# msg7086/x265-Yuuki-Asuna

Measured on AMD Instinct MI355X. Metric: encoded fps + bit-exact check, 4K preset=slow, 1/2/4/8 MI355X vs host AVX2, higher is better.
Workload: dtype u8; 1 GPU; 3840x2160 8-bit closed-loop frame pipeline (tier T2): lookahead -> exhaustive +-57 ME, 85 PUs/CTU -> subme 3 -> MC + DCT/quant/recon qp 27 -> deblock -> SAO (rdo) -> border -> next reference; parallelism=none (1 GPU), ctus_per_frame=2040

## Files before the change

### include/x265hip.h

```cpp
#ifndef X265HIP_H
#define X265HIP_H

#include <stdint.h>
#include <stddef.h>

#ifdef __cplusplus
extern "C" {
#endif

#define X265HIP_ME_PUS_PER_CTU 85
#define X265HIP_OK            0
#define X265HIP_ENODEV       -1
#define X265HIP_EINVAL       -2
#define X265HIP_EUNSUPPORTED -3
#define X265HIP_EBUSY        -4

const char* x265hip_version(void);
int x265hip_stream_release(void* stream);
const char* x265hip_last_error(void);
int         x265hip_device_count(void);
int         x265hip_init(int device);
#define X265HIP_WAIT_BLOCK 0
#define X265HIP_WAIT_SPIN  1
int         x265hip_set_wait_policy(int policy);
// ... 39 lines not shown
static inline size_t x265hip_surf_ctu_bytes(int surf_format, int range)
{
    const size_t nc = (size_t)(2 * range + 1), recs = nc * ((nc + 3) >> 2);
    if (surf_format == X265HIP_SURF_I32) return recs * X265HIP_SURF_GROUP_BYTES_I32;
    if (surf_format == X265HIP_SURF_PACKED_B) return ((recs + 63) >> 6) * X265HIP_SURF_BLOCK_BYTES_PACKED;
    return recs * X265HIP_SURF_GROUP_BYTES_PACKED;
}
int x265hip_me_fullsearch(const x265hip_me_params* p, void* stream);
int x265hip_me_best_reset(uint64_t* best, size_t count, void* stream);
const char* x265hip_me_minima_kernel_name(int depth, int range);
void x265hip_me_env_refresh(void);

typedef struct x265hip_subpel_params
{
    int depth;
    int width, height;
    int range;
    int subme;
    const void* fenc;  intptr_t fenc_stride;
    const void* fref;  intptr_t fref_stride;
    const uint64_t* best_in;
    const uint16_t* cost_q;  int qoff;
    void* out;
    const void* phase_planes;  intptr_t phase_plane_samples;
} x265hip_subpel_params;
int x265hip_subpel_refine(const x265hip_subpel_params* p, void* stream);

typedef struct x265hip_subpel_chroma
{
    const void* fenc_cb; const void* fenc_cr; intptr_t fenc_stride_c;
    const void* fref_cb; const void* fref_cr; intptr_t fref_stride_c;
} x265hip_subpel_chroma;
int x265hip_subpel_refine_chroma(const x265hip_subpel_params* p, const x265hip_subpel_chroma* c, void* stream);

#define X265HIP_TU_INTRA_SLICE 1
#define X265HIP_TU_SIGN_HIDE   2
typedef struct x265hip_tu_tables
{
    const int32_t* quant_coeff;
    const int32_t* dequant_coeff;
    const uint16_t* nr_offset;
    uint32_t* nr_residual_sum;
    int16_t* dct_coeff_out;
    int32_t* delta_u_out;
    int64_t* rdoq_cost_uncoded;
    int64_t* rdoq_cg_cost;
    int16_t* rdoq_levels;
    uint32_t* rdoq_num_sig;
    int16_t* fenc_dct_out;
    int64_t psy_scale;
} x265hip_tu_tables;
typedef struct x265hip_recon_params
{
    int depth;
    int width, height;
    int level;
    int qp, intra_slice;
    const void* fenc;  intptr_t fenc_stride;
    const void* fref;  intptr_t fref_stride;
    void* recon;       intptr_t recon_stride;
    const void* mv;
    int16_t* levels; uint32_t* num_sig; uint64_t* dist;
    const x265hip_tu_tables* tables;
    const int8_t* qp_map;
} x265hip_recon_params;
int x265hip_inter_recon(const x265hip_recon_params* p, void* stream);
// ... 787 lines not shown
```

### x265-yuuki-asuna_amd/csrc/subpel_kernels.hip

```cpp
#include "common.h"
#include "tile_interp.h"

namespace x265hip {

struct SubpelArgs
{
    const uint8_t* fenc; long fencStrideB;
    const uint8_t* fref; long frefStrideB;
    int ctusW, range, depth;
    const unsigned long long* bestIn;
    const uint16_t* costQ; int qoff;
    int hpelIters, hpelDirs, qpelIters, qpelDirs, hpelSatd;
    int2* out;
    const uint8_t* planes; long planeBytes;
};

struct SubpelChromaArgs
{
    const uint8_t* fencC[2]; long fencStrideCB;
    const uint8_t* frefC[2]; long frefStrideCB;
};

__constant__ int16_t kSpLumaTaps[4][8] = {
    { 0, 0, 0, 64, 0, 0, 0, 0 }, { -1, 4, -10, 58, 17, -5, 1, 0 },
    { -1, 4, -11, 40, 40, -11, 4, -1 }, { 0, 1, -5, 17, 58, -10, 4, -1 } };
__constant__ int kSpSquare1[9][2] = { { 0, 0 }, { 0, -1 }, { 0, 1 }, { -1, 0 }, { 1, 0 }, { -1, -1 }, { -1, 1 }, { 1, -1 }, { 1, 1 } };

constexpr int SP_MARGIN = 7;

__device__ __forceinline__ int sp_clip16(int v, int maxVal)
{
    const int16_t s = (int16_t)v;
    return s < 0 ? 0 : (s > maxVal ? maxVal : s);
}

struct SpShared
{
    int cost[64][9];
    int best[64], qx[64], qy[64], ix[64], iy[64], state[64];
};

template <typename Px, int LEVEL> struct SpGeom
{
    static constexpr int BPP = sizeof(Px);
    static constexpr int N = 8 << LEVEL, NPU = 64 >> (2 * LEVEL);
    static constexpr int TSHIFT = 2 * LEVEL + 2, NTILES = 1 << TSHIFT, TPR = N >> 2;
    static constexpr int PW = N + 2 * SP_MARGIN + 1;
// ... 318 lines not shown
        {
            const int qx0 = sh.qx[tid], qy0 = sh.qy[tid];
            if (isRem)
                sh.best[tid] = sh.cost[tid][0] + mvcost(qx0, qy0);
            else
            {
                int bcost = sh.best[tid], bdir = 0;
                for (int i = 1; i <= last; i++)
                {
                    const int c = sh.cost[tid][i] + mvcost(qx0 + kSpSquare1[i][0] * step, qy0 + kSpSquare1[i][1] * step);
                    if (c < bcost) { bcost = c; bdir = i; }
                }
                sh.best[tid] = bcost;
                if (bdir) { sh.qx[tid] = qx0 + kSpSquare1[bdir][0] * step; sh.qy[tid] = qy0 + kSpSquare1[bdir][1] * step; }
                else sh.state[tid] = 2;
            }
        }
        if (G::NTILES == 256) { __syncthreads(); if (tid < 9) sh.cost[0][tid] = 0; }
        __syncthreads();
    }
    if (tid < NPU)
    {
        int bcost = sh.best[tid];
        if (sh.state[tid] == 0) bcost = mvcost(sh.qx[tid], sh.qy[tid]);
        a.out[(size_t)ctu * 85 + G::LBASE + tid] = make_int2(bcost, (sh.qx[tid] & 0xffff) | (sh.qy[tid] << 16));
    }
}

template <typename Px, bool PL = false>
__global__ void __launch_bounds__(256) subpel_refine_kernel(SubpelArgs a)
{
    extern __shared__ __attribute__((aligned(16))) uint8_t smemRaw[];
    __shared__ SpShared sh;
    switch (blockIdx.y)
    {
    case 0: subpel_level<Px, 0, PL>(a, smemRaw, sh); break;
    case 1: subpel_level<Px, 1, PL>(a, smemRaw, sh); break;
    case 2: subpel_level<Px, 2, PL>(a, smemRaw, sh); break;
    default: subpel_level<Px, 3, PL>(a, smemRaw, sh); break;
    }
}

template <typename Px, bool PL>
__global__ void __launch_bounds__(256) subpel_refine_chroma_kernel(SubpelArgs a, SubpelChromaArgs ca)
{
    extern __shared__ __attribute__((aligned(16))) uint8_t smemRaw[];
    __shared__ SpShared sh;
    switch (blockIdx.y)
    {
    case 0: subpel_level<Px, 0, PL, true>(a, smemRaw, sh, ca); break;
    case 1: subpel_level<Px, 1, PL, true>(a, smemRaw, sh, ca); break;
    case 2: subpel_level<Px, 2, PL, true>(a, smemRaw, sh, ca); break;
    default: subpel_level<Px, 3, PL, true>(a, smemRaw, sh, ca); break;
    }
}

}

using namespace x265hip;

extern "C" int x265hip_subpel_refine(const x265hip_subpel_params* p, void* stream)
{
    return x265hip_subpel_refine_chroma(p, nullptr, stream);
}

extern "C" int x265hip_subpel_refine_chroma(const x265hip_subpel_params* p, const x265hip_subpel_chroma* c, void* stream)
{
    if (!p || !p->fenc || !p->fref || !p->best_in || !p->cost_q || !p->out) { set_error("subpel_refine: NULL operand"); return X265HIP_EINVAL; }
    if ((p->width & 63) || (p->height & 63) || p->width <= 0 || p->height <= 0) { set_error("subpel_refine: width/height must be multiples of 64"); return X265HIP_EINVAL; }
    if (p->depth != 8 && p->depth != 10 && p->depth != 12) { set_error("subpel_refine: depth %d", p->depth); return X265HIP_EINVAL; }
    if (p->subme < 0 || p->subme > 7) { set_error("subpel_refine: subme %d out of [0,7]", p->subme); return X265HIP_EINVAL; }
    if (p->phase_planes && p->phase_plane_samples <= 0) { set_error("subpel_refine: phase_plane_samples"); return X265HIP_EINVAL; }
    if (c)
    {
        if (!c->fenc_cb || !c->fenc_cr || !c->fref_cb || !c->fref_cr) { set_error("subpel_refine_chroma: NULL chroma plane"); return X265HIP_EINVAL; }
        if (c->fenc_stride_c <= 0 || c->fref_stride_c <= 0) { set_error("subpel_refine_chroma: chroma strides must be positive"); return X265HIP_EINVAL; }
    }
    int rc = ensure_device();
    if (rc) return rc;
    static const int wl[8][5] = { { 1, 4, 0, 4, 0 }, { 1, 4, 1, 4, 0 }, { 1, 4, 1, 4, 1 }, { 2, 4, 1, 4, 1 },
                                  { 2, 4, 2, 4, 1 }, { 1, 8, 1, 8, 1 }, { 2, 8, 1, 8, 1 }, { 2, 8, 2, 8, 1 } };
    const int bpp = p->depth == 8 ? 1 : 2;
    SubpelArgs a;
    a.fenc = (const uint8_t*)p->fenc; a.fencStrideB = (long)p->fenc_stride * bpp;
    a.fref = (const uint8_t*)p->fref; a.frefStrideB = (long)p->fref_stride * bpp;
    a.ctusW = p->width / 64; a.range = p->range; a.depth = p->depth;
    a.bestIn = (const unsigned long long*)p->best_in; a.costQ = p->cost_q; a.qoff = p->qoff;
    a.hpelIters = wl[p->subme][0]; a.hpelDirs = wl[p->subme][1]; a.qpelIters = wl[p->subme][2]; a.qpelDirs = wl[p->subme][3]; a.hpelSatd = wl[p->subme][4];
    a.out = (int2*)p->out;
    a.planes = (const uint8_t*)p->phase_planes; a.planeBytes = (long)p->phase_plane_samples * bpp;
    const int nctu = a.ctusW * (p->height / 64);
    hipStream_t s = (hipStream_t)stream;
    const size_t lds = (size_t)(bpp == 1 ? SpGeom<uint8_t, 0>::PSZ : SpGeom<uint16_t, 0>::PSZ) * 64 * bpp;
    static_assert(SpGeom<uint8_t, 0>::PSZ * 64 >= SpGeom<uint8_t, 1>::PSZ * 16 && SpGeom<uint8_t, 0>::PSZ * 64 >= SpGeom<uint8_t, 2>::PSZ * 4
                  && SpGeom<uint8_t, 0>::PSZ * 64 >= SpGeom<uint8_t, 3>::PSZ, "level 0 is the largest");
    static_assert(SpGeom<uint16_t, 0>::PSZ * 64 >= SpGeom<uint16_t, 1>::PSZ * 16 && SpGeom<uint16_t, 0>::PSZ * 64 >= SpGeom<uint16_t, 2>::PSZ * 4
                  && SpGeom<uint16_t, 0>::PSZ * 64 >= SpGeom<uint16_t, 3>::PSZ, "level 0 is the largest");
    if (c && p->subme >= 3)
    {
        SubpelChromaArgs ca;
        ca.fencC[0] = (const uint8_t*)c->fenc_cb; ca.fencC[1] = (const uint8_t*)c->fenc_cr; ca.fencStrideCB = (long)c->fenc_stride_c * bpp;
        ca.frefC[0] = (const uint8_t*)c->fref_cb; ca.frefC[1] = (const uint8_t*)c->fref_cr; ca.frefStrideCB = (long)c->fref_stride_c * bpp;
        if (a.planes)
        {
            if (p->depth == 8) hipLaunchKernelGGL((subpel_refine_chroma_kernel<uint8_t, true>), dim3(nctu, 4), dim3(256), 0, s, a, ca);
            else hipLaunchKernelGGL((subpel_refine_chroma_kernel<uint16_t, true>), dim3(nctu, 4), dim3(256), 0, s, a, ca);
        }
        else if (p->depth == 8)
            hipLaunchKernelGGL((subpel_refine_chroma_kernel<uint8_t, false>), dim3(nctu, 4), dim3(256), lds, s, a, ca);
        else
        {
            static bool attrC = false;
            if (!attrC) { X265HIP_TRY(hipFuncSetAttribute((const void*)subpel_refine_chroma_kernel<uint16_t, false>, hipFuncAttributeMaxDynamicSharedMemorySize, (int)lds)); attrC = true; }
            hipLaunchKernelGGL((subpel_refine_chroma_kernel<uint16_t, false>), dim3(nctu, 4), dim3(256), lds, s, a, ca);
        }
    }
    else if (a.planes)
    {
        if (p->depth == 8) hipLaunchKernelGGL((subpel_refine_kernel<uint8_t, true>), dim3(nctu, 4), dim3(256), 0, s, a);
        else hipLaunchKernelGGL((subpel_refine_kernel<uint16_t, true>), dim3(nctu, 4), dim3(256), 0, s, a);
    }
    else if (p->depth == 8)
        hipLaunchKernelGGL(subpel_refine_kernel<uint8_t>, dim3(nctu, 4), dim3(256), lds, s, a);
    else
    {
        static bool attr = false;
        if (!attr) { X265HIP_TRY(hipFuncSetAttribute((const void*)subpel_refine_kernel<uint16_t>, hipFuncAttributeMaxDynamicSharedMemorySize, (int)lds)); attr = true; }
        hipLaunchKernelGGL(subpel_refine_kernel<uint16_t>, dim3(nctu, 4), dim3(256), lds, s, a);
    }
    X265HIP_TRY(hipGetLastError());
    return 0;
}
```

### x265-yuuki-asuna_amd/hipabi.py

```python
from __future__ import annotations

import ctypes
import os

_HERE = os.path.dirname(os.path.abspath(__file__))
LIB_PATH = os.path.join(_HERE, "libx265hip.so")

CMP_SAD, CMP_SATD, CMP_SA8D, CMP_SSE_PP, CMP_PSY_COST = range(5)

_lib = None


class X265HipError(RuntimeError):
    pass


class MEParams(ctypes.Structure):
    _fields_ = [
        ("depth", ctypes.c_int), ("width", ctypes.c_int), ("height", ctypes.c_int), ("range", ctypes.c_int),
        ("fenc", ctypes.c_void_p), ("fenc_stride", ctypes.c_ssize_t),
        ("fref", ctypes.c_void_p), ("fref_stride", ctypes.c_ssize_t),
        ("surf", ctypes.c_void_p), ("best", ctypes.c_void_p),
        ("cost_x", ctypes.c_void_p), ("cost_y", ctypes.c_void_p),
        ("surf_format", ctypes.c_int),
# ... 208 lines not shown
def exported_symbols():
    import re
    hdr = os.path.join(os.path.dirname(_HERE), "include", "x265hip.h")
    text = open(hdr).read()
    inline = set(re.findall(r"static inline [^\n(]*\b(x265hip_[a-z0-9_]+)\s*\(", text))
    return sorted(set(re.findall(r"\b(x265hip_[a-z0-9_]+)\s*\(", text)) - inline)


def current_stream() -> int:
    import torch
    return torch.cuda.current_stream().cuda_stream


def _p(t):
    return None if t is None else t.data_ptr()


def me_fullsearch(depth, width, height, rng, fenc, fenc_stride, fref, fref_stride,
                  surf=None, best=None, cost_x=None, cost_y=None,
                  fenc_off=0, fref_off=0, stream=None, surf_format=SURF_I32, centres=None):
    es = 1 if depth == 8 else 2
    p = MEParams()
    p.surf_format = surf_format
    p.depth, p.width, p.height, p.range = depth, width, height, rng
    p.fenc, p.fenc_stride = fenc.data_ptr() + fenc_off * es, fenc_stride
    p.fref, p.fref_stride = fref.data_ptr() + fref_off * es, fref_stride
    p.surf, p.best = _p(surf), _p(best)
    p.cost_x, p.cost_y = _p(cost_x), _p(cost_y)
    p.centres = _p(centres)
    s = current_stream() if stream is None else stream
    check(lib().x265hip_me_fullsearch(ctypes.byref(p), s), "x265hip_me_fullsearch")


def subpel_refine(depth, width, height, rng, subme, fenc, fenc_stride, fref, fref_stride, best_in, cost_q, qoff, out,
                  fenc_off=0, fref_off=0, stream=None, phase_planes=None, chroma=None):
    es = 1 if depth == 8 else 2
    p = SubpelParams()
    p.depth, p.width, p.height, p.range, p.subme = depth, width, height, rng, subme
    p.fenc, p.fenc_stride = fenc.data_ptr() + fenc_off * es, fenc_stride
    p.fref, p.fref_stride = fref.data_ptr() + fref_off * es, fref_stride
    p.best_in, p.cost_q, p.qoff, p.out = best_in.data_ptr(), cost_q.data_ptr(), qoff, out.data_ptr()
    if phase_planes is not None:
        p.phase_planes, p.phase_plane_samples = phase_planes.data_ptr() + fref_off * es, fref.numel() * fref.element_size() // es
    s = current_stream() if stream is None else stream
    if chroma is not None:
        c = SubpelChroma()
        c.fenc_cb, c.fenc_cr = (t.data_ptr() + chroma["fenc_org"] * es for t in chroma["fenc"])
        c.fref_cb, c.fref_cr = (t.data_ptr() + chroma["fref_org"] * es for t in chroma["fref"])
        c.fenc_stride_c, c.fref_stride_c = chroma["fenc_stride"], chroma["fref_stride"]
        f = lib().x265hip_subpel_refine_chroma
        f.argtypes = [ctypes.POINTER(SubpelParams), ctypes.POINTER(SubpelChroma), ctypes.c_void_p]
        check(f(ctypes.byref(p), ctypes.byref(c), s), "x265hip_subpel_refine_chroma")
        return
    f = lib().x265hip_subpel_refine
    f.argtypes = [ctypes.POINTER(SubpelParams), ctypes.c_void_p]
    check(f(ctypes.byref(p), s), "x265hip_subpel_refine")


def bidir_decide(depth, width, height, level, fenc, fenc_stride, fref0, fref1, fref_stride, mv0, mv1, cost_q, qoff, dir_cost, dir_out, mv0_out, mv1_out,
                 ref0=None, ref1=None, cost_out=None, ref_ids=(0, 1), fenc_off=0, fref_off=0, phase_planes=None, stream=None, chroma=None):
    es = 1 if depth == 8 else 2
    p = BidirParams()
    p.depth, p.width, p.height, p.level = depth, width, height, level
    p.fenc, p.fenc_stride = fenc.data_ptr() + fenc_off * es, fenc_stride
    p.fref0, p.fref1, p.fref_stride = fref0.data_ptr() + fref_off * es, fref1.data_ptr() + fref_off * es, fref_stride
    p.mv0, p.mv1, p.cost_q, p.qoff = mv0.data_ptr(), mv1.data_ptr(), cost_q.data_ptr(), qoff
    p.dir_cost[0], p.dir_cost[1], p.dir_cost[2] = (int(c) for c in dir_cost)
    p.ref_id0, p.ref_id1 = ref_ids
    if phase_planes is not None:
        p.phase_planes0, p.phase_planes1 = (t.data_ptr() + fref_off * es for t in phase_planes)
        p.phase_plane_samples = fref0.numel() * fref0.element_size() // es
    p.dir, p.ref0, p.ref1 = dir_out.data_ptr(), _p(ref0), _p(ref1)
    p.mv0_out, p.mv1_out, p.cost_out = mv0_out.data_ptr(), mv1_out.data_ptr(), _p(cost_out)
    s = current_stream() if stream is None else stream
    if chroma is not None:
        c = BidirChroma()
        c.fenc_cb, c.fenc_cr = (t.data_ptr() + chroma["fenc_org"] * es for t in chroma["fenc"])
        c.fref0_cb, c.fref0_cr = (t.data_ptr() + chroma["fref_org"] * es for t in chroma["fref0"])
        c.fref1_cb, c.fref1_cr = (t.data_ptr() + chroma["fref_org"] * es for t in chroma["fref1"])
        c.fenc_stride_c, c.fref_stride_c = chroma["fenc_stride"], chroma["fref_stride"]
        f = lib().x265hip_bidir_decide_chroma
        f.argtypes = [ctypes.POINTER(BidirParams), ctypes.POINTER(BidirChroma), ctypes.c_void_p]
# ... 994 lines not shown
```

### x265-yuuki-asuna_amd/pipeline.py

```python
from __future__ import annotations

import numpy as np

from . import frames as F
from . import hipabi

LEVEL_SIZES = (8, 16, 32, 64)
LEVEL_PUS = (64, 16, 4, 1)
LEVEL_BASE = (0, 64, 80, 84)
PUS_PER_CTU = 85


class DevicePicture:

    def __init__(self, img: np.ndarray, device, cb: np.ndarray = None, cr: np.ndarray = None):
        import torch
        buf, self.stride, self.org, self.w64, self.h64 = F.pad_plane(img)
        self.depth = 8 if img.dtype == np.uint8 else 10

        def up(b):
            return torch.from_numpy(b if b.dtype == np.uint8 else b.view(np.int16)).to(device)
        self.t = up(buf)
        self.host = buf
        self.c, self.c_host, self.stride_c, self.org_c = None, None, 0, 0
# ... 134 lines not shown
            out["surf"] = int(sum(self.level_view(l)[0].sum(dtype=torch.int64).item() for l in range(4)))
        return out


class SubpelRefine:

    def __init__(self, ms: MotionSearch, subme: int, device, lam=4.0, phase_planes=False, chroma_satd=False):
        import torch
        self.ms, self.subme = ms, subme
        self.chroma_satd = bool(chroma_satd)
        self.use_planes, self.planes = bool(phase_planes), None
        cq, self.qoff = F.qpel_cost_table(ms.range, lam)
        self.cost_q_host = cq
        self.cost_q = torch.from_numpy(cq.view(np.int16)).to(device)
        self.out = torch.zeros(ms.nctu * PUS_PER_CTU * 2, dtype=torch.int32, device=device)

    def part(self, ms_part, ctu_row0):
        import copy
        o = copy.copy(self)
        o.ms, o.parent = ms_part, self
        c0 = (ms_part.w64 // 64) * ctu_row0
        o.out = self.out[c0 * PUS_PER_CTU * 2:(c0 + ms_part.nctu) * PUS_PER_CTU * 2]
        return o

    def prepare(self, ref: DevicePicture):
        import torch
        if not self.use_planes:
            return
        nb = ref.t.numel() * ref.t.element_size()
        if self.planes is None or self.planes.numel() != 15 * nb:
            self.planes = torch.empty(15 * nb, dtype=torch.uint8, device=ref.t.device)
        hipabi.phase_planes(self.ms.depth, ref.t, 0, self.planes, ref.stride, nb // (ref.stride * (1 if self.ms.depth == 8 else 2)))

    def run(self, cur: DevicePicture, ref: DevicePicture, prepared=False):
        ms = self.ms
        if not prepared:
            self.prepare(ref)
        planes = getattr(self, "parent", self).planes if self.use_planes else None
        chroma = None
        if self.chroma_satd:
            if cur.c is None or ref.c is None:
                raise ValueError("SubpelRefine(chroma_satd=True) needs pictures with chroma planes")
            if (4 * ms.range + 6 + 7) // 8 + 6 > min(F.CHROMA_MARGIN_X, F.CHROMA_MARGIN_Y):
                raise ValueError(f"SubpelRefine(chroma_satd=True): range {ms.range} reaches past the {F.CHROMA_MARGIN_Y}-row chroma margin")
            chroma = dict(fenc=cur.c, fenc_stride=cur.stride_c, fenc_org=cur.org_c, fref=ref.c, fref_stride=ref.stride_c, fref_org=ref.org_c)
        hipabi.subpel_refine(ms.depth, ms.w64, ms.h64, ms.range, self.subme, cur.t, cur.stride, ref.t, ref.stride,
                             ms.best, self.cost_q, self.qoff, self.out, fenc_off=cur.org, fref_off=ref.org, phase_planes=planes, chroma=chroma)

    def checksum(self):
        return {"subpel": int(self.out.to(dtype=__import__("torch").int64).sum().item())}


class FrameParallel:

    def __init__(self, rank: int, world: int):
        self.rank, self.world = rank, world

    def frame_index(self, step: int) -> int:
        return step * self.world + self.rank

    def reference_owner(self) -> int:
        return self.world - 1

    def exchange(self, ref_plane, newest_plane):
        if isinstance(ref_plane, (list, tuple)):
            for r, n in zip(ref_plane, newest_plane):
                self.exchange(r, n)
            return
        if self.world == 1:
            ref_plane.copy_(newest_plane)
            return
        import torch.distributed as dist
        if self.rank == self.reference_owner():
            ref_plane.copy_(newest_plane)
        dist.broadcast(ref_plane, src=self.reference_owner())


class DistTransport:

    def __init__(self, rank, world, stage_through_host=False):
# ... 395 lines not shown
```

### x265-yuuki-asuna_amd/stages.py

```python
from __future__ import annotations

import ctypes
import os

import numpy as np

from . import hipabi
from .pipeline import PUS_PER_CTU, DevicePicture


ReconParams = hipabi.ReconParams


def _tu_part(stage, ctu_row0, ctu_rows):
    import copy
    o = copy.copy(stage)
    cw = stage.w64 // 64
    c0, o.nctu, o.h64 = cw * ctu_row0, cw * ctu_rows, ctu_rows * 64
    nb, nn = stage.nblk, stage.n * stage.n
    o.levels = stage.levels[c0 * nb * nn:(c0 + o.nctu) * nb * nn]
    o.num_sig = stage.num_sig[c0 * nb:(c0 + o.nctu) * nb]
    o.dist = stage.dist[c0 * nb:(c0 + o.nctu) * nb]
    if stage.qp_map is not None:
        o.qp_map = stage.qp_map[ctu_row0 * 8 * (stage.w64 // 8):(ctu_row0 + ctu_rows) * 8 * (stage.w64 // 8)]
# ... 190 lines not shown

def extend_border(plane, pic: DevicePicture, stream=None, chroma=False):
    from . import frames as F
    es = 1 if pic.depth == 8 else 2
    s = hipabi.current_stream() if stream is None else stream
    f = hipabi.lib().x265hip_extend_border
    f.argtypes = [ctypes.c_void_p, ctypes.c_ssize_t, ctypes.c_int, ctypes.c_int, ctypes.c_int, ctypes.c_int, ctypes.c_int, ctypes.c_void_p]
    if chroma:
        hipabi.check(f(plane.data_ptr() + pic.org_c * es, pic.stride_c, pic.w64 // 2, pic.h64 // 2, F.CHROMA_MARGIN_X, F.CHROMA_MARGIN_Y, pic.depth, s),
                     "x265hip_extend_border")
        return
    hipabi.check(f(plane.data_ptr() + pic.org * es, pic.stride, pic.w64, pic.h64, F.MARGIN_X, F.MARGIN_Y, pic.depth, s),
                 "x265hip_extend_border")


class BorderPlane(ctypes.Structure):
    _fields_ = [("pic", ctypes.c_void_p), ("stride", ctypes.c_ssize_t), ("width", ctypes.c_int), ("height", ctypes.c_int), ("margin_x", ctypes.c_int),
                ("margin_top", ctypes.c_int), ("margin_bottom", ctypes.c_int)]


def extend_border_picture(planes, pic: DevicePicture, stream=None, top=True, bottom=True):
    from . import frames as F
    es = 1 if pic.depth == 8 else 2
    s = hipabi.current_stream() if stream is None else stream
    arr = (BorderPlane * len(planes))()
    arr[0] = BorderPlane(planes[0].data_ptr() + pic.org * es, pic.stride, pic.w64, pic.h64, F.MARGIN_X, F.MARGIN_Y if top else 0, F.MARGIN_Y if bottom else 0)
    for i in range(1, len(planes)):
        arr[i] = BorderPlane(planes[i].data_ptr() + pic.org_c * es, pic.stride_c, pic.w64 // 2, pic.h64 // 2, F.CHROMA_MARGIN_X,
                             F.CHROMA_MARGIN_Y if top else 0, F.CHROMA_MARGIN_Y if bottom else 0)
    f = hipabi.lib().x265hip_extend_border_planes
    f.argtypes = [ctypes.POINTER(BorderPlane), ctypes.c_int, ctypes.c_int, ctypes.c_void_p]
    hipabi.check(f(arr, len(planes), pic.depth, s), "x265hip_extend_border_planes")


_CHROMA_SCALE = list(range(30)) + [29, 30, 31, 32, 33, 33, 34, 34, 35, 35, 36, 36, 37, 37] + list(range(38, 52)) + [51] * 12


def chroma_quant_qp(qp, depth, offset=0):
    bd = 6 * (depth - 8)
    q = min(max(qp - bd + offset, -bd), 57)
    if q >= 30:
        q = _CHROMA_SCALE[q]
    return q + bd


class CuQpMaps:

    def __init__(self, w64, h64, depth, level, device, qg_size=16, qp_min=0, qp_max=51, cb_qp_offset=0, cr_qp_offset=0):
        import torch
        self.w64, self.h64, self.depth, self.level, self.qg_size = w64, h64, depth, level, qg_size
        self.qp_min, self.qp_max, self.cb_qp_offset, self.cr_qp_offset = qp_min, qp_max, cb_qp_offset, cr_qp_offset
        cells = (h64 // 8) * (w64 // 8)
        self.cu_qp = torch.zeros(cells, dtype=torch.int8, device=device)
        self.tu_qp = torch.zeros(3 * cells, dtype=torch.int8, device=device).view(3, cells)
        self.cu_qp_host = self.tu_qp_host = None

    def run(self, base_qp, qp_offsets=None):
        import torch
        cu, tu = hipabi.cu_qp_maps(self.depth, self.w64, self.h64, self.level, self.qg_size, base_qp, qp_offsets, self.qp_min, self.qp_max,
                                   self.cb_qp_offset, self.cr_qp_offset)
        return self.load(cu, tu)

    def load(self, cu, tu):
        import torch
        self.cu_qp_host, self.tu_qp_host = np.ascontiguousarray(cu, dtype=np.int8), np.ascontiguousarray(tu, dtype=np.int8)
        self.cu_qp.copy_(torch.from_numpy(self.cu_qp_host.reshape(-1)))
# ... 295 lines not shown
        integral = None
        if self.method == hipabi.ME_SEA:
            integral = hipabi.sea_integral(self.depth, ref.t, ref.stride, ref.org, self.w64, self.h64, F.MARGIN_X, F.MARGIN_Y, planes=self.planes)
            self.planes = integral[0]
        hipabi.me_search(self.depth, cur.t, cur.stride, cur.org, ref.t, ref.stride, ref.org, self.method, self.subme, r,
                         self.cost_q, self.qoff, (-r, -r), (r, r), self.jobs, self.njobs, integral=integral)
        o = self.out.view(-1, 2)
        o[:, 0] = self.jobs[:, 8]
        o[:, 1] = (self.jobs[:, 6] & 0xffff) | (self.jobs[:, 7] << 16)

    def checksum(self):
        import torch
        return {"subpel": int(self.out.to(dtype=torch.int64).sum().item())}


class FramePipeline:

    def __init__(self, w64, h64, depth, device, rng=57, subme=2, level=2, qp=27, want_surf=True, packed=False, lookahead=None,
                 search="full", deblock=False, sao=False, lookahead_cost_batch=0, chroma=False, sao_apply=False, sign_hide=False,
                 subpel_planes=False, parallel_planes=False, split=1, sao_rdo=None, chroma_satd=False):
        import torch
        from .pipeline import MotionSearch, SubpelRefine
        self.depth = depth
        self.parallel = bool(parallel_planes)
        self.pstreams = None
        self._spare_ready = None
        self.schedule2 = os.environ.get("X265HIP_PAR_SCHEDULE", "2") != "1"
        self.split = max(1, min(int(split), h64 // 64))
        self.parts = None
        self.fuse_sao = os.environ.get("X265HIP_FUSE_SAO", "1") != "0"
        self.fuse_sao_parallel = os.environ.get("X265HIP_FUSE_SAO", "1") == "2"
        self.la_after_search = os.environ.get("X265HIP_LA_AFTER_ME", "1") == "1"
        self.prep_next_to_search = os.environ.get("X265HIP_PREP_OVERLAP", "0") == "1"
        self.ms = MotionSearch(w64, h64, rng, depth, device, want_surf=want_surf and search == "full", want_best=True, packed=packed)
        if chroma_satd and search != "full":
            raise ValueError("FramePipeline: chroma_satd needs search='full' (the pattern-search step is luma only)")
        if chroma_satd and not chroma:
            raise ValueError("FramePipeline: chroma_satd needs chroma=True")
        self.sp = SubpelRefine(self.ms, subme, device, phase_planes=subpel_planes, chroma_satd=chroma_satd)
        self.ps = None
        if search != "full":
            method = {"dia": hipabi.ME_DIA, "hex": hipabi.ME_HEX, "umh": hipabi.ME_UMH, "star": hipabi.ME_STAR, "sea": hipabi.ME_SEA}[search]
            self.ps = PatternSearch(w64, h64, depth, method, subme, rng, device)
        self.tu_flags = hipabi.TU_SIGN_HIDE if sign_hide else 0
        self.rc = InterRecon(self.ms.nctu, w64, h64, depth, level, qp, device, intra_slice=self.tu_flags)
        self.la = Lookahead(lookahead[0], lookahead[1], depth, device) if lookahead else None
        self.lcb = lookahead_cost_batch if lookahead else 0
        if self.lcb:
            self.ring = [self.la] + [Lookahead(lookahead[0], lookahead[1], depth, device) for _ in range(2 * self.lcb)]
            self.lc = [LookaheadCost(self.la, device) for _ in range(self.lcb)]
            self.side = torch.cuda.Stream(device=device)
            self.frame_no, self.pending, self.read_done = 0, [], {}
            self.device, self.tables = device, {}
            nring = len(self.ring)
            for j in range(nring):
                self._table(tuple(((j * self.lcb + 1 + i) % nring, (j * self.lcb + i) % nring) for i in range(self.lcb)))
            torch.cuda.synchronize()
        self.db = Deblock(w64, h64, depth, level, max(qp - 6 * (depth - 8), 0), device) if deblock else None
        self.sao = Sao(w64, h64, depth, device) if sao else None
        self.recon = None
        self.chroma = chroma
        self.qp = qp
        self.recon_c, self.out, self.out_c = None, None, None
        if chroma:
            qpc = chroma_quant_qp(qp, depth)
            self.rc_c = [InterReconChroma(self.ms.nctu, w64, h64, depth, level, qpc, device, intra_slice=self.tu_flags) for _ in range(2)]
# ... 222 lines not shown
        for i, st in enumerate((sCb, sCr)):
            if self.fuse_sao_parallel or self.sao_rdo is not None:
                st.wait_event(ev_sao)
            with torch.cuda.stream(st):
                if not self.fuse_sao_parallel and self.sao_rdo is None:
                    self.sao_c[i].stats(None, self.recon_c[i], cur.stride_c, cur.org_c, src_plane=cur.c[i])
                    self.sao_c[i].decide()
                    self.sao_c[i].apply(self.recon_c[i], cur.stride_c, cur.org_c, self.out_c[i])
                border(self.out_c[i], True)
                e = torch.cuda.Event(); e.record(st); done.append(e)
        if self.la is not None:
            e = torch.cuda.Event(); e.record(sLa); done.append(e)
        for e in done:
            main.wait_event(e)
        self.final, self.final_c = self.out, self.out_c
        return self.final

    def _run_parallel2(self, cur, ref, main, sC):
        import torch
        ms = self.ms
        if self._spare_ready:
            ms.swap_best()
        else:
            ms.reset()
        if self.prep_next_to_search:
            ev0 = torch.cuda.Event(); ev0.record(main)
            sC.wait_event(ev0)
            with torch.cuda.stream(sC):
                self.sp.prepare(ref)
                ev_pl = torch.cuda.Event(); ev_pl.record(sC)
        ms.search(cur, ref)
        if self.prep_next_to_search:
            main.wait_event(ev_pl)
        self.sp.run(cur, ref, prepared=self.prep_next_to_search)
        mv = self.sp.out
        ev_mv = torch.cuda.Event(); ev_mv.record(main)
        self.rc.run(cur, ref, self.recon, mv)
        sC.wait_event(ev_mv)
        with torch.cuda.stream(sC):
            InterReconChroma.run_pair(self.rc_c, cur.c, ref.c, self.recon_c, cur.stride_c, cur.org_c, mv)
        self.db.run(self.recon, cur, mv, self.rc.num_sig)
        ev_bs = torch.cuda.Event(); ev_bs.record(main)
        planes = self._sao_planes(cur)
        sC.wait_event(ev_bs)
        with torch.cuda.stream(sC):
            hipabi.deblock_chroma(self.depth, self.recon_c[0], self.recon_c[1], cur.stride_c, cur.org_c, cur.w64, cur.h64,
                                  self.db.bs_ver, self.db.bs_hor, self.db.qp, qp_map=self.db.qp_map)
            hipabi.sao_planes(self.depth, [dict(q, out=None) for q in planes[1:3]])
            ev_cstats = torch.cuda.Event(); ev_cstats.record(sC)
            ms.reset_spare()
            self._spare_ready = True
            if self.la is not None:
                self.la.run(cur)
            ev_side = torch.cuda.Event(); ev_side.record(sC)
        hipabi.sao_planes(self.depth, [dict(planes[0], out=None)])
        main.wait_event(ev_cstats)
        self._sao_rdo()
        hipabi.sao_apply_planes(self.depth, planes)
        if os.environ.get("X265HIP_BORDER_PLANES", "1") == "0":
            extend_border(self.out, cur)
            for i in range(2):
                extend_border(self.out_c[i], cur, chroma=True)
        else:
            extend_border_picture([self.out] + list(self.out_c), cur)
        main.wait_event(ev_side)
        self.final, self.final_c = self.out, self.out_c
        return self.final

    def swap_output(self, spare):
        if self.final is not self.out or self.out is None or (self.chroma and self.final_c is not self.out_c):
            return None
        outs = self.final_planes()
        self.out = spare[0]
        if self.chroma:
            self.out_c = list(spare[1:3])
        return outs

    def _search_to_recon_in_parts(self, cur, ref, main, sCb, sCr, start):
        import torch
        if self.parts is None:
            rows = self.ms.h64 // 64
            cuts = [rows * k // self.split for k in range(self.split + 1)]
            self.parts = []
            for r0, r1 in zip(cuts[:-1], cuts[1:]):
                msp = self.ms.part(r0, r1 - r0)
                self.parts.append((r0, r1 - r0, msp, self.sp.part(msp, r0), self.rc.part(r0, r1 - r0), [q.part(r0, r1 - r0) for q in self.rc_c]))
        sY = self.pstreams[3]
        sY.wait_event(start)
        with torch.cuda.stream(sY):
            self.sp.prepare(ref)
        last = len(self.parts) - 1
        for k, (r0, n, msp, spp, rcp, rcc) in enumerate(self.parts):
            c, r = cur.band_view(r0, n), ref.band_view(r0, n)
            msp.search(c, r)
            ev_me = torch.cuda.Event(); ev_me.record(main)
            st = main if k == last else sY
            if k == last:
                main.wait_stream(sY)
# ... 633 lines not shown
```

Baseline: 638.4 frames/s.

## Run only recon-critical subpel level on main stream, defer other levels to side stream

Subpel refinement can now be launched for a chosen subset of partition levels, through a level mask and a per-block level lookup table. The frame pipeline runs only the level that inter recon consumes on the main stream, and runs the remaining three levels on the side stream after lookahead (default "after"). Alternative placements are available through an environment variable. This is meant to take most of the subpel work off the critical path so it overlaps with chroma, SAO and border work. Per-mask launches also size dynamic LDS to the largest selected level, which may improve occupancy, but the change adds extra launches and more load on the side stream.

```diff
diff --git a/include/x265hip.h b/include/x265hip.h
--- a/include/x265hip.h
+++ b/include/x265hip.h
@@ -95,6 +95,8 @@
     const void* fref_cb; const void* fref_cr; intptr_t fref_stride_c;
 } x265hip_subpel_chroma;
 int x265hip_subpel_refine_chroma(const x265hip_subpel_params* p, const x265hip_subpel_chroma* c, void* stream);
+
+int x265hip_subpel_refine_levels(const x265hip_subpel_params* p, const x265hip_subpel_chroma* c, unsigned level_mask, void* stream);
 
 #define X265HIP_TU_INTRA_SLICE 1
 #define X265HIP_TU_SIGN_HIDE   2
diff --git a/x265-yuuki-asuna_amd/csrc/subpel_kernels.hip b/x265-yuuki-asuna_amd/csrc/subpel_kernels.hip
--- a/x265-yuuki-asuna_amd/csrc/subpel_kernels.hip
+++ b/x265-yuuki-asuna_amd/csrc/subpel_kernels.hip
@@ -13,6 +13,7 @@
     int hpelIters, hpelDirs, qpelIters, qpelDirs, hpelSatd;
     int2* out;
     const uint8_t* planes; long planeBytes;
+    unsigned levelTab;
 };
 
 struct SubpelChromaArgs
@@ -397,7 +398,7 @@
 {
     extern __shared__ __attribute__((aligned(16))) uint8_t smemRaw[];
     __shared__ SpShared sh;
-    switch (blockIdx.y)
+    switch ((a.levelTab >> (2 * blockIdx.y)) & 3)
     {
     case 0: subpel_level<Px, 0, PL>(a, smemRaw, sh); break;
     case 1: subpel_level<Px, 1, PL>(a, smemRaw, sh); break;
@@ -411,7 +412,7 @@
 {
     extern __shared__ __attribute__((aligned(16))) uint8_t smemRaw[];
     __shared__ SpShared sh;
-    switch (blockIdx.y)
+    switch ((a.levelTab >> (2 * blockIdx.y)) & 3)
     {
     case 0: subpel_level<Px, 0, PL, true>(a, smemRaw, sh, ca); break;
     case 1: subpel_level<Px, 1, PL, true>(a, smemRaw, sh, ca); break;
@@ -420,6 +421,103 @@
     }
 }
 
+template <typename Px, int LEVEL, bool PL>
+__global__ void __launch_bounds__(256) subpel_refine_level_kernel(SubpelArgs a)
+{
+    extern __shared__ __attribute__((aligned(16))) uint8_t smemRaw[];
+    __shared__ SpShared sh;
+    subpel_level<Px, LEVEL, PL>(a, smemRaw, sh);
+}
+
+template <typename Px, int LEVEL, bool PL>
+__global__ void __launch_bounds__(256) subpel_refine_chroma_level_kernel(SubpelArgs a, SubpelChromaArgs ca)
+{
+    extern __shared__ __attribute__((aligned(16))) uint8_t smemRaw[];
+    __shared__ SpShared sh;
+    subpel_level<Px, LEVEL, PL, true>(a, smemRaw, sh, ca);
+}
+
+template <typename Px>
+static size_t sp_patch_bytes(const unsigned mask)
+{
+    const size_t per[4] = { (size_t)SpGeom<Px, 0>::PSZ * 64, (size_t)SpGeom<Px, 1>::PSZ * 16, (size_t)SpGeom<Px, 2>::PSZ * 4, (size_t)SpGeom<Px, 3>::PSZ };
+    size_t n = 0;
+    for (int l = 0; l < 4; l++)
+        if (((mask >> l) & 1) && per[l] > n) n = per[l];
+    return n * sizeof(Px);
+}
+
+constexpr size_t SP_LDS_DEFAULT_MAX = 65536;
+
+template <typename Px, int LEVEL, bool PL, bool CH>
+static hipError_t sp_launch_level(const SubpelArgs& a, const SubpelChromaArgs& ca, const int nctu, const size_t lds, hipStream_t s)
+{
+    static bool attr = false;
+    if constexpr (CH)
+    {
+        if (lds > SP_LDS_DEFAULT_MAX && !attr)
+        {
+            const hipError_t e = hipFuncSetAttribute((const void*)subpel_refine_chroma_level_kernel<Px, LEVEL, PL>, hipFuncAttributeMaxDynamicSharedMemorySize, (int)lds);
+            if (e != hipSuccess) return e;
+            attr = true;
+        }
+        hipLaunchKernelGGL((subpel_refine_chroma_level_kernel<Px, LEVEL, PL>), dim3(nctu, 1), dim3(256), lds, s, a, ca);
+    }
+    else
+    {
+        if (lds > SP_LDS_DEFAULT_MAX && !attr)
+        {
+            const hipError_t e = hipFuncSetAttribute((const void*)subpel_refine_level_kernel<Px, LEVEL, PL>, hipFuncAttributeMaxDynamicSharedMemorySize, (int)lds);
+            if (e != hipSuccess) return e;
+            attr = true;
+        }
+        hipLaunchKernelGGL((subpel_refine_level_kernel<Px, LEVEL, PL>), dim3(nctu, 1), dim3(256), lds, s, a);
+    }
+    return hipSuccess;
+}
+
+template <typename Px, bool PL, bool CH>
+static hipError_t sp_launch(SubpelArgs a, const SubpelChromaArgs& ca, const unsigned mask, const int nctu, hipStream_t s)
+{
+    const size_t lds = PL ? 0 : sp_patch_bytes<Px>(mask);
+    if (!(mask & (mask - 1)))
+    {
+        switch (mask)
+        {
+        case 1: return sp_launch_level<Px, 0, PL, CH>(a, ca, nctu, lds, s);
+        case 2: return sp_launch_level<Px, 1, PL, CH>(a, ca, nctu, lds, s);
+        case 4: return sp_launch_level<Px, 2, PL, CH>(a, ca, nctu, lds, s);
+        default: return sp_launch_level<Px, 3, PL, CH>(a, ca, nctu, lds, s);
+        }
+    }
+    int rows = 0;
+    a.levelTab = 0;
+    for (unsigned l = 0; l < 4; l++)
+        if ((mask >> l) & 1) a.levelTab |= l << (2 * rows++);
+    static bool attr = false;
+    if constexpr (CH)
+    {
+        if (lds > SP_LDS_DEFAULT_MAX && !attr)
+        {
+            const hipError_t e = hipFuncSetAttribute((const void*)subpel_refine_chroma_kernel<Px, PL>, hipFuncAttributeMaxDynamicSharedMemorySize, (int)lds);
+            if (e != hipSuccess) return e;
+            attr = true;
+        }
+        hipLaunchKernelGGL((subpel_refine_chroma_kernel<Px, PL>), dim3(nctu, rows), dim3(256), lds, s, a, ca);
+    }
+    else
+    {
+        if (lds > SP_LDS_DEFAULT_MAX && !attr)
+        {
+            const hipError_t e = hipFuncSetAttribute((const void*)subpel_refine_kernel<Px, PL>, hipFuncAttributeMaxDynamicSharedMemorySize, (int)lds);
+            if (e != hipSuccess) return e;
+            attr = true;
+        }
+        hipLaunchKernelGGL((subpel_refine_kernel<Px, PL>), dim3(nctu, rows), dim3(256), lds, s, a);
+    }
+    return hipSuccess;
+}
+
 }
 
 using namespace x265hip;
@@ -430,12 +528,18 @@
 }
 
 extern "C" int x265hip_subpel_refine_chroma(const x265hip_subpel_params* p, const x265hip_subpel_chroma* c, void* stream)
+{
+    return x265hip_subpel_refine_levels(p, c, 15, stream);
+}
+
+extern "C" int x265hip_subpel_refine_levels(const x265hip_subpel_params* p, const x265hip_subpel_chroma* c, unsigned level_mask, void* stream)
 {
     if (!p || !p->fenc || !p->fref || !p->best_in || !p->cost_q || !p->out) { set_error("subpel_refine: NULL operand"); return X265HIP_EINVAL; }
     if ((p->width & 63) || (p->height & 63) || p->width <= 0 || p->height <= 0) { set_error("subpel_refine: width/height must be multiples of 64"); return X265HIP_EINVAL; }
     if (p->depth != 8 && p->depth != 10 && p->depth != 12) { set_error("subpel_refine: depth %d", p->depth); return X265HIP_EINVAL; }
     if (p->subme < 0 || p->subme > 7) { set_error("subpel_refine: subme %d out of [0,7]", p->subme); return X265HIP_EINVAL; }
     if (p->phase_planes && p->phase_plane_samples <= 0) { set_error("subpel_refine: phase_plane_samples"); return X265HIP_EINVAL; }
+    if (level_mask == 0 || level_mask > 15) { set_error("subpel_refine_levels: level_mask %u out of [1,15]", level_mask); return X265HIP_EINVAL; }
     if (c)
     {
         if (!c->fenc_cb || !c->fenc_cr || !c->fref_cb || !c->fref_cr) { set_error("subpel_refine_chroma: NULL chroma plane"); return X265HIP_EINVAL; }
@@ -454,45 +558,25 @@
     a.hpelIters = wl[p->subme][0]; a.hpelDirs = wl[p->subme][1]; a.qpelIters = wl[p->subme][2]; a.qpelDirs = wl[p->subme][3]; a.hpelSatd = wl[p->subme][4];
     a.out = (int2*)p->out;
     a.planes = (const uint8_t*)p->phase_planes; a.planeBytes = (long)p->phase_plane_samples * bpp;
+    a.levelTab = 0xe4;
     const int nctu = a.ctusW * (p->height / 64);
     hipStream_t s = (hipStream_t)stream;
-    const size_t lds = (size_t)(bpp == 1 ? SpGeom<uint8_t, 0>::PSZ : SpGeom<uint16_t, 0>::PSZ) * 64 * bpp;
-    static_assert(SpGeom<uint8_t, 0>::PSZ * 64 >= SpGeom<uint8_t, 1>::PSZ * 16 && SpGeom<uint8_t, 0>::PSZ * 64 >= SpGeom<uint8_t, 2>::PSZ * 4
-                  && SpGeom<uint8_t, 0>::PSZ * 64 >= SpGeom<uint8_t, 3>::PSZ, "level 0 is the largest");
-    static_assert(SpGeom<uint16_t, 0>::PSZ * 64 >= SpGeom<uint16_t, 1>::PSZ * 16 && SpGeom<uint16_t, 0>::PSZ * 64 >= SpGeom<uint16_t, 2>::PSZ * 4
-                  && SpGeom<uint16_t, 0>::PSZ * 64 >= SpGeom<uint16_t, 3>::PSZ, "level 0 is the largest");
-    if (c && p->subme >= 3)
-    {
-        SubpelChromaArgs ca;
+    SubpelChromaArgs ca = SubpelChromaArgs();
+    const bool ch = c && p->subme >= 3;
+    if (ch)
+    {
         ca.fencC[0] = (const uint8_t*)c->fenc_cb; ca.fencC[1] = (const uint8_t*)c->fenc_cr; ca.fencStrideCB = (long)c->fenc_stride_c * bpp;
         ca.frefC[0] = (const uint8_t*)c->fref_cb; ca.frefC[1] = (const uint8_t*)c->fref_cr; ca.frefStrideCB = (long)c->fref_stride_c * bpp;
-        if (a.planes)
-        {
-            if (p->depth == 8) hipLaunchKernelGGL((subpel_refine_chroma_kernel<uint8_t, true>), dim3(nctu, 4), dim3(256), 0, s, a, ca);
-            else hipLaunchKernelGGL((subpel_refine_chroma_kernel<uint16_t, true>), dim3(nctu, 4), dim3(256), 0, s, a, ca);
-        }
-        else if (p->depth == 8)
-            hipLaunchKernelGGL((subpel_refine_chroma_kernel<uint8_t, false>), dim3(nctu, 4), dim3(256), lds, s, a, ca);
-        else
-        {
-            static bool attrC = false;
-            if (!attrC) { X265HIP_TRY(hipFuncSetAttribute((const void*)subpel_refine_chroma_kernel<uint16_t, false>, hipFuncAttributeMaxDynamicSharedMemorySize, (int)lds)); attrC = true; }
-            hipLaunchKernelGGL((subpel_refine_chroma_kernel<uint16_t, false>), dim3(nctu, 4), dim3(256), lds, s, a, ca);
-        }
-    }
-    else if (a.planes)
-    {
-        if (p->depth == 8) hipLaunchKernelGGL((subpel_refine_kernel<uint8_t, true>), dim3(nctu, 4), dim3(256), 0, s, a);
-        else hipLaunchKernelGGL((subpel_refine_kernel<uint16_t, true>), dim3(nctu, 4), dim3(256), 0, s, a);
-    }
-    else if (p->depth == 8)
-        hipLaunchKernelGGL(subpel_refine_kernel<uint8_t>, dim3(nctu, 4), dim3(256), lds, s, a);
+    }
+    const bool pl = a.planes != nullptr;
+    hipError_t e;
+    if (bpp == 1)
+        e = ch ? (pl ? sp_launch<uint8_t, true, true>(a, ca, level_mask, nctu, s) : sp_launch<uint8_t, false, true>(a, ca, level_mask, nctu, s))
+               : (pl ? sp_launch<uint8_t, true, false>(a, ca, level_mask, nctu, s) : sp_launch<uint8_t, false, false>(a, ca, level_mask, nctu, s));
     else
-    {
-        static bool attr = false;
-        if (!attr) { X265HIP_TRY(hipFuncSetAttribute((const void*)subpel_refine_kernel<uint16_t>, hipFuncAttributeMaxDynamicSharedMemorySize, (int)lds)); attr = true; }
-        hipLaunchKernelGGL(subpel_refine_kernel<uint16_t>, dim3(nctu, 4), dim3(256), lds, s, a);
-    }
+        e = ch ? (pl ? sp_launch<uint16_t, true, true>(a, ca, level_mask, nctu, s) : sp_launch<uint16_t, false, true>(a, ca, level_mask, nctu, s))
+               : (pl ? sp_launch<uint16_t, true, false>(a, ca, level_mask, nctu, s) : sp_launch<uint16_t, false, false>(a, ca, level_mask, nctu, s));
+    X265HIP_TRY(e);
     X265HIP_TRY(hipGetLastError());
     return 0;
 }
diff --git a/x265-yuuki-asuna_amd/hipabi.py b/x265-yuuki-asuna_amd/hipabi.py
--- a/x265-yuuki-asuna_amd/hipabi.py
+++ b/x265-yuuki-asuna_amd/hipabi.py
@@ -264,8 +264,22 @@
     check(lib().x265hip_me_fullsearch(ctypes.byref(p), s), "x265hip_me_fullsearch")
 
 
+def subpel_level_mask(levels):
+    if isinstance(levels, int):
+        mask = levels
+    else:
+        mask = 0
+        for l in levels:
+            if not 0 <= int(l) <= 3:
+                raise ValueError(f"subpel level {l} out of [0,3]")
+            mask |= 1 << int(l)
+    if not 1 <= mask <= 15:
+        raise ValueError(f"subpel level mask {mask} out of [1,15]")
+    return mask
+
+
 def subpel_refine(depth, width, height, rng, subme, fenc, fenc_stride, fref, fref_stride, best_in, cost_q, qoff, out,
-                  fenc_off=0, fref_off=0, stream=None, phase_planes=None, chroma=None):
+                  fenc_off=0, fref_off=0, stream=None, phase_planes=None, chroma=None, levels=None):
     es = 1 if depth == 8 else 2
     p = SubpelParams()
     p.depth, p.width, p.height, p.range, p.subme = depth, width, height, rng, subme
@@ -275,11 +289,18 @@
     if phase_planes is not None:
         p.phase_planes, p.phase_plane_samples = phase_planes.data_ptr() + fref_off * es, fref.numel() * fref.element_size() // es
     s = current_stream() if stream is None else stream
+    c = None
     if chroma is not None:
         c = SubpelChroma()
         c.fenc_cb, c.fenc_cr = (t.data_ptr() + chroma["fenc_org"] * es for t in chroma["fenc"])
         c.fref_cb, c.fref_cr = (t.data_ptr() + chroma["fref_org"] * es for t in chroma["fref"])
         c.fenc_stride_c, c.fref_stride_c = chroma["fenc_stride"], chroma["fref_stride"]
+    if levels is not None:
+        f = lib().x265hip_subpel_refine_levels
+        f.argtypes = [ctypes.POINTER(SubpelParams), ctypes.POINTER(SubpelChroma), ctypes.c_uint, ctypes.c_void_p]
+        check(f(ctypes.byref(p), None if c is None else ctypes.byref(c), subpel_level_mask(levels), s), "x265hip_subpel_refine_levels")
+        return
+    if c is not None:
         f = lib().x265hip_subpel_refine_chroma
         f.argtypes = [ctypes.POINTER(SubpelParams), ctypes.POINTER(SubpelChroma), ctypes.c_void_p]
         check(f(ctypes.byref(p), ctypes.byref(c), s), "x265hip_subpel_refine_chroma")
diff --git a/x265-yuuki-asuna_amd/pipeline.py b/x265-yuuki-asuna_amd/pipeline.py
--- a/x265-yuuki-asuna_amd/pipeline.py
+++ b/x265-yuuki-asuna_amd/pipeline.py
@@ -190,7 +190,7 @@
             self.planes = torch.empty(15 * nb, dtype=torch.uint8, device=ref.t.device)
         hipabi.phase_planes(self.ms.depth, ref.t, 0, self.planes, ref.stride, nb // (ref.stride * (1 if self.ms.depth == 8 else 2)))
 
-    def run(self, cur: DevicePicture, ref: DevicePicture, prepared=False):
+    def run(self, cur: DevicePicture, ref: DevicePicture, prepared=False, levels=None):
         ms = self.ms
         if not prepared:
             self.prepare(ref)
@@ -203,7 +203,7 @@
                 raise ValueError(f"SubpelRefine(chroma_satd=True): range {ms.range} reaches past the {F.CHROMA_MARGIN_Y}-row chroma margin")
             chroma = dict(fenc=cur.c, fenc_stride=cur.stride_c, fenc_org=cur.org_c, fref=ref.c, fref_stride=ref.stride_c, fref_org=ref.org_c)
         hipabi.subpel_refine(ms.depth, ms.w64, ms.h64, ms.range, self.subme, cur.t, cur.stride, ref.t, ref.stride,
-                             ms.best, self.cost_q, self.qoff, self.out, fenc_off=cur.org, fref_off=ref.org, phase_planes=planes, chroma=chroma)
+                             ms.best, self.cost_q, self.qoff, self.out, fenc_off=cur.org, fref_off=ref.org, phase_planes=planes, chroma=chroma, levels=levels)
 
     def checksum(self):
         return {"subpel": int(self.out.to(dtype=__import__("torch").int64).sum().item())}
diff --git a/x265-yuuki-asuna_amd/stages.py b/x265-yuuki-asuna_amd/stages.py
--- a/x265-yuuki-asuna_amd/stages.py
+++ b/x265-yuuki-asuna_amd/stages.py
@@ -246,6 +246,8 @@
     f.argtypes = [ctypes.POINTER(BorderPlane), ctypes.c_int, ctypes.c_int, ctypes.c_void_p]
     hipabi.check(f(arr, len(planes), pic.depth, s), "x265hip_extend_border_planes")
 
+
+SUBPEL_DEFER_DEFAULT = "after"
 
 _CHROMA_SCALE = list(range(30)) + [29, 30, 31, 32, 33, 33, 34, 34, 35, 35, 36, 36, 37, 37] + list(range(38, 52)) + [51] * 12
 
@@ -607,6 +609,10 @@
         self.fuse_sao_parallel = os.environ.get("X265HIP_FUSE_SAO", "1") == "2"
         self.la_after_search = os.environ.get("X265HIP_LA_AFTER_ME", "1") == "1"
         self.prep_next_to_search = os.environ.get("X265HIP_PREP_OVERLAP", "0") == "1"
+        defer = os.environ.get("X265HIP_SUBPEL_DEFER", "1")
+        if defer not in ("0", "1", "before", "after", "mv"):
+            raise ValueError(f"X265HIP_SUBPEL_DEFER={defer}: 0, 1, before, after or mv")
+        self.subpel_defer = {"0": None, "1": SUBPEL_DEFER_DEFAULT}.get(defer, defer)
         self.ms = MotionSearch(w64, h64, rng, depth, device, want_surf=want_surf and search == "full", want_best=True, packed=packed)
         if chroma_satd and search != "full":
             raise ValueError("FramePipeline: chroma_satd needs search='full' (the pattern-search step is luma only)")
@@ -895,9 +901,18 @@
         ms.search(cur, ref)
         if self.prep_next_to_search:
             main.wait_event(ev_pl)
-        self.sp.run(cur, ref, prepared=self.prep_next_to_search)
+        defer = self.subpel_defer
+        rest = [l for l in range(4) if l != self.rc.level]
+        self.sp.run(cur, ref, prepared=self.prep_next_to_search, levels=(self.rc.level,) if defer else None)
         mv = self.sp.out
         ev_mv = torch.cuda.Event(); ev_mv.record(main)
+        ev_rest = None
+        if defer == "mv":
+            sD = self.pstreams[1]
+            sD.wait_event(ev_mv)
+            with torch.cuda.stream(sD):
+                self.sp.run(cur, ref, prepared=True, levels=rest)
+                ev_rest = torch.cuda.Event(); ev_rest.record(sD)
         self.rc.run(cur, ref, self.recon, mv)
         sC.wait_event(ev_mv)
         with torch.cuda.stream(sC):
@@ -913,8 +928,12 @@
             ev_cstats = torch.cuda.Event(); ev_cstats.record(sC)
             ms.reset_spare()
             self._spare_ready = True
+            if defer == "before":
+                self.sp.run(cur, ref, prepared=True, levels=rest)
             if self.la is not None:
                 self.la.run(cur)
+            if defer == "after":
+                self.sp.run(cur, ref, prepared=True, levels=rest)
             ev_side = torch.cuda.Event(); ev_side.record(sC)
         hipabi.sao_planes(self.depth, [dict(planes[0], out=None)])
         main.wait_event(ev_cstats)
@@ -927,6 +946,8 @@
         else:
             extend_border_picture([self.out] + list(self.out_c), cur)
         main.wait_event(ev_side)
+        if ev_rest is not None:
+            main.wait_event(ev_rest)
         self.final, self.final_c = self.out, self.out_c
         return self.final
 
```

After: 657.2 frames/s, median of 6. 1.03x the previous value.
